# aiola-lab/whisper-medusa

Measured on AMD Instinct MI355X. Metric: decoded_tokens_per_sec, higher is better.
Workload: dtype bf16 + fp16 decoder GEMM operands (one plane; fp32 accumulate)

## Files before the change

whisper-medusa_amd/csrc/wm_decoder.hip:

```cpp
#include "wm_internal.h"
#include <algorithm>
#include <cstdlib>
#include <type_traits>
#include "wm_skinny_gemm.h"
#include "wm_select.h"

__global__ void k_embed(float* __restrict__ h, const bf16_t* __restrict__ tok_emb, const float* __restrict__ pos_emb,
                        const int* __restrict__ base, const int* __restrict__ tok_src, int tok_stride, int use_base_off,
                        int Mper, int d, int V, int Tmax, const int* __restrict__ depth,
                        const int4* __restrict__ rowinfo = nullptr, const int* __restrict__ ids = nullptr, int ids_stride = 0,
                        const float* __restrict__ gnext = nullptr, bf16_t* __restrict__ xo = nullptr, size_t xplane = 0,
                        float2* __restrict__ stats = nullptr, int sld = 0)
{
    const int row = blockIdx.x;
    int s = row / Mper, r = row - s * Mper;
    bool base_row = false;
    int b0;
    if (rowinfo) {
        const int4 ri = rowinfo[row];
        if (ri.w == 0) return;
        s = ri.x; r = ri.y; b0 = ri.z; base_row = ri.w == 1;
    } else {
        b0 = base[s];
    }
// ... 374 lines not shown
    typedef unsigned long long u64;
    float M = -INFINITY, L = 0.f; float4 acc = make_float4(0.f, 0.f, 0.f, 0.f);

    for (int sp = sp0; sp < sp1; ++sp) {
        AttnAcc st;
        st.m_run = -INFINITY; st.l_run = 0.f;
#pragma unroll
        for (int dt = 0; dt < 4; ++dt) st.o[dt] = f32x4_t{0.f, 0.f, 0.f, 0.f};
        if (CROSS) {
            const int nkb = (sp + 1) * 256 + w * 64, nkend = (sp + 1 < sp1) ? min(S, nkb + 64) : 0;
            if (aw && kb < kend) attn_block64(st, kv_widen(c0), kv_widen(c1), qhi, qlo, kb, g, limit, kb + 32 < kend);
            if constexpr (KV8) {
                if (aw && nkb < nkend) kv_load8(c0, kp8, vp8, nkb, c, g, lane);
                if (aw && nkb + 32 < nkend) kv_load8(c1, kp8, vp8, nkb + 32, c, g, lane);
            } else {
                if (aw && nkb < nkend) kv_load<NT>(c0, kp, vp, nkb, c, g, lane);
                if (aw && nkb + 32 < nkend) kv_load<NT>(c1, kp, vp, nkb + 32, c, g, lane);
            }
            kb = nkb; kend = nkend;
        } else {
            for (; kb < kend; kb += 128) {
                const bool second = CROSS ? false : ((kb >> 7) & 1);
                if constexpr (!KV8) {
                    if (kb + 128 < kend) { if (second) kv_load<NT>(c0, kp, vp, kb + 128, c, g, lane); else kv_load<NT>(c1, kp, vp, kb + 128, c, g, lane); }
                    if (second) attn_step(st, c1, qhi, qlo, kb, g, limit, b0, anc); else attn_step(st, c0, qhi, qlo, kb, g, limit, b0, anc);
                }
            }
        }
        const float m_run = st.m_run, l_run = st.l_run;
        const f32x4_t (&o)[4] = st.o;
        if (aw) {
            if (g == 0) { s_m[w][c] = m_run; s_l[w][c] = l_run; }
#pragma unroll
            for (int dt = 0; dt < 4; ++dt)
                *reinterpret_cast<float4*>(&s_o[w][c][dt * 16 + 4 * g]) = make_float4(o[dt][0], o[dt][1], o[dt][2], o[dt][3]);
        }
        __syncthreads();
        M = -INFINITY; L = 0.f; acc = make_float4(0.f, 0.f, 0.f, 0.f);
        if (qr < rows) {
            M = fmaxf(fmaxf(s_m[0][qr], s_m[1][qr]), fmaxf(s_m[2][qr], s_m[3][qr]));
#pragma unroll
            for (int ww = 0; ww < 4; ++ww) {
                const float e = (s_m[ww][qr] == -INFINITY) ? 0.f : __expf(s_m[ww][qr] - M);
                L += s_l[ww][qr] * e;
                const float4 ov = *reinterpret_cast<const float4*>(&s_o[ww][qr][ch]);
                acc.x += ov.x * e; acc.y += ov.y * e; acc.z += ov.z * e; acc.w += ov.w * e;
            }
        }
        if (!CROSS) break;
        if (qr < rows) {
            *reinterpret_cast<float4*>(&s_part[sp - sp0][qr][ch]) = acc;
            if (ch == 0) { s_part[sp - sp0][qr][64] = M; s_part[sp - sp0][qr][65] = L; }
            if (gx > 1) {
                u64* pd = reinterpret_cast<u64*>(po + (((size_t)row * H + hd) * NS + sp) * 64 + ch);
                __hip_atomic_store(pd, ((u64)__float_as_uint(acc.y) << 32) | __float_as_uint(acc.x), __ATOMIC_RELAXED, __HIP_MEMORY_SCOPE_AGENT);
                __hip_atomic_store(pd + 1, ((u64)__float_as_uint(acc.w) << 32) | __float_as_uint(acc.z), __ATOMIC_RELAXED, __HIP_MEMORY_SCOPE_AGENT);
                if (ch == 0)
                    __hip_atomic_store(reinterpret_cast<u64*>(ml + (((size_t)row * H + hd) * NS + sp) * 2),
                                       ((u64)__float_as_uint(L) << 32) | __float_as_uint(M), __ATOMIC_RELAXED, __HIP_MEMORY_SCOPE_AGENT);
            }
        }
        if (sp + 1 < sp1) __syncthreads();
    }
    TL_MID
    if (!CROSS) {
        if (qr < rows) {
            const float inv = 1.0f / L;
            const size_t oi = packed_index(row, hd * 64 + ch, K32);
            act_st4(xout + oi, xout + xplane + oi, make_float4(acc.x * inv, acc.y * inv, acc.z * inv, acc.w * inv));
        }
        TL_END
        return;
    }
    if (gx > 1) {
        asm volatile("s_waitcnt vmcnt(0)" ::: "memory");
        __syncthreads();
        if (threadIdx.x == 0) {
            const int t = __hip_atomic_fetch_add(ticket + blockIdx.z * H + hd, 1, __ATOMIC_RELAXED, __HIP_MEMORY_SCOPE_AGENT);
            const int last = (t == gx - 1);
            if (last) __hip_atomic_store(ticket + blockIdx.z * H + hd, 0, __ATOMIC_RELAXED, __HIP_MEMORY_SCOPE_AGENT);
            s_last = last;
        }
        __syncthreads();
        if (!s_last) { TL_END return; }
    } else __syncthreads();
    if (qr < rows) {
        float ms[WM_XATTN_NS_MAX], ls[WM_XATTN_NS_MAX]; float4 ov[WM_XATTN_NS_MAX];
        if (gx > 1) {
            const u64* mlp = reinterpret_cast<const u64*>(ml + ((size_t)row * H + hd) * NS * 2);
            const u64* op = reinterpret_cast<const u64*>(po + ((size_t)row * H + hd) * NS * 64 + ch);
            u64 rml[WM_XATTN_NS_MAX], ro0[WM_XATTN_NS_MAX], ro1[WM_XATTN_NS_MAX];
#pragma unroll
            for (int sp = 0; sp < WM_XATTN_NS_MAX; ++sp) {
                const int spc = min(sp, NS - 1);
                rml[sp] = __hip_atomic_load(mlp + spc, __ATOMIC_RELAXED, __HIP_MEMORY_SCOPE_AGENT);
                ro0[sp] = __hip_atomic_load(op + (size_t)spc * 32, __ATOMIC_RELAXED, __HIP_MEMORY_SCOPE_AGENT);
                ro1[sp] = __hip_atomic_load(op + (size_t)spc * 32 + 1, __ATOMIC_RELAXED, __HIP_MEMORY_SCOPE_AGENT);
            }
#pragma unroll
            for (int sp = 0; sp < WM_XATTN_NS_MAX; ++sp) {
                ms[sp] = __uint_as_float((unsigned)rml[sp]); ls[sp] = __uint_as_float((unsigned)(rml[sp] >> 32));
                ov[sp] = make_float4(__uint_as_float((unsigned)ro0[sp]), __uint_as_float((unsigned)(ro0[sp] >> 32)),
                                     __uint_as_float((unsigned)ro1[sp]), __uint_as_float((unsigned)(ro1[sp] >> 32)));
            }
        } else {
#pragma unroll
            for (int sp = 0; sp < WM_XATTN_NS_MAX; ++sp) {
                const int spc = min(sp, NS - 1);
                ms[sp] = s_part[spc][qr][64]; ls[sp] = s_part[spc][qr][65];
                ov[sp] = *reinterpret_cast<const float4*>(&s_part[spc][qr][ch]);
            }
        }
        float Mx = -INFINITY;
#pragma unroll
        for (int sp = 0; sp < WM_XATTN_NS_MAX; ++sp) if (sp < NS) Mx = fmaxf(Mx, ms[sp]);
        float Lt = 0.f; float4 o4 = make_float4(0.f, 0.f, 0.f, 0.f);
#pragma unroll
        for (int sp = 0; sp < WM_XATTN_NS_MAX; ++sp) {
            if (sp < NS) {
                const float e = (ms[sp] == -INFINITY) ? 0.f : __expf(ms[sp] - Mx);
                Lt += ls[sp] * e;
                o4.x += ov[sp].x * e; o4.y += ov[sp].y * e; o4.z += ov[sp].z * e; o4.w += ov[sp].w * e;
            }
        }
        const float inv = vsc / Lt;
        const size_t oi = packed_index(row, hd * 64 + ch, K32);
        act_st4(xout + oi, xout + xplane + oi, make_float4(o4.x * inv, o4.y * inv, o4.z * inv, o4.w * inv));
    }
    TL_END
}


__device__ __forceinline__ void sib_block_pop(float (&tv)[6], int (&ti)[6], float* sv, int* si, int tid, float& mx, int& mi)
{
    const int lane = tid & 63, w = tid >> 6;
    mx = tv[0]; mi = ti[0];
#pragma unroll
    for (int o = 32; o > 0; o >>= 1) {
        const float ov = __shfl_xor(mx, o, 64); const int oi = __shfl_xor(mi, o, 64);
        if (ov > mx || (ov == mx && oi < mi)) { mx = ov; mi = oi; }
    }
    __syncthreads();
    if (lane == 0) { sv[w] = mx; si[w] = mi; }
    __syncthreads();
    mx = sv[0]; mi = si[0];
#pragma unroll
    for (int q = 1; q < 4; ++q) if (sv[q] > mx || (sv[q] == mx && si[q] < mi)) { mx = sv[q]; mi = si[q]; }
    if (ti[0] == mi && mi != 0x7fffffff) {
#pragma unroll
        for (int q = 0; q < 5; ++q) { tv[q] = tv[q + 1]; ti[q] = ti[q + 1]; }
        tv[5] = -INFINITY; ti[5] = 0x7fffffff;
    }
}
__device__ __forceinline__ void sib_insert(float (&tv)[6], int (&ti)[6], float v, int vi)
{
    if (v > tv[5] || (v == tv[5] && vi < ti[5])) {
#pragma unroll
        for (int j = 0; j < 6; ++j)
            if (v > tv[j] || (v == tv[j] && vi < ti[j])) { const float fv = tv[j]; const int fi = ti[j]; tv[j] = v; ti[j] = vi; v = fv; vi = fi; }
    }
}

template <bool NEED_Z, bool TS>
__device__ __forceinline__ void
select1_body(const float* __restrict__ logits, const GenDev& gp, const unsigned char* __restrict__ mask, const float* __restrict__ exppen,
             const int* __restrict__ L, int rps, float* __restrict__ part1, const int4* __restrict__ rowinfo, float2* __restrict__ sibpart,
             const TsDev& ts, int ts_verify)
{
    __shared__ float sv[4]; __shared__ int si[4]; __shared__ float sz[4];
    const int row = blockIdx.y, sp = blockIdx.x;
    int s = row / rps, ri_i = row - s * rps;
    const bool sibrow = sibpart != nullptr && row - s * rps == 1;
    if (rowinfo) {
        const int4 ri = rowinfo[row];
        if (ri.w != 2) return;
        s = ri.x; ri_i = ri.y;
    }
    const int tid = threadIdx.x, lane = tid & 63, w = tid >> 6;
    const int cur_len = L[s];
    const float* x = logits + (size_t)row * gp.Vpad;
    const int per = (gp.V + SEL_SP - 1) / SEL_SP, n0 = sp * per, n1 = min(gp.V, n0 + per);
    int4 rec = make_int4(0, 0, 0, 0);
    if (TS) rec = ts_row_record(gp, ts, ts_verify, s, ri_i, cur_len);
    extern __shared__ unsigned rp_sh[];
    const bool rp = TS && ts.rp != 0;
    if (rp) rp_build(ts, rp_row_prefix(ts, ts_verify, s, ri_i, cur_len), n0, n1, -1, gp.V, rp_sh, tid, 256);
    auto pl = [&](int n) {
        float v = x[n];
        if (rp) v = rp_pen(v, n, n0, ts, rp_sh);
        v = proc_logit(v, n, cur_len, gp, mask, exppen);
        if (TS) v = ts_mask(v, n, rec, gp, ts);
        if (rp && rp_banned(n, n0, gp.V, rp_sh)) v = -INFINITY;
        return v;
    };
    float mx = -INFINITY; int mi = 0x7fffffff;
    if (sibrow) {
        float tv[6]; int ti[6];
#pragma unroll
        for (int j = 0; j < 6; ++j) { tv[j] = -INFINITY; ti[j] = 0x7fffffff; }
        for (int n = n0 + tid; n < n1; n += 256) sib_insert(tv, ti, pl(n), n);
        float2* mine = sibpart + ((size_t)s * SEL_SP + sp) * 6;
        float m0 = -INFINITY; int i0 = 0x7fffffff;
        for (int j = 0; j < 6; ++j) {
            float pm; int pi;
            sib_block_pop(tv, ti, sv, si, tid, pm, pi);
            if (j == 0) { m0 = pm; i0 = pi; }
            if (tid == 0) mine[j] = make_float2(pm, __int_as_float(pi));
        }
        __syncthreads();
        mx = m0; mi = i0;
    } else if (!TS) {
        for (int n = n0 + tid; n < n1; n += 256) {
            const float v = proc_logit(x[n], n, cur_len, gp, mask, exppen);
            if (v > mx || (v == mx && n < mi)) { mx = v; mi = n; }
        }
#pragma unroll
        for (int o = 32; o > 0; o >>= 1) {
            const float ov = __shfl_xor(mx, o, 64); const int oi = __shfl_xor(mi, o, 64);
            if (ov > mx || (ov == mx && oi < mi)) { mx = ov; mi = oi; }
        }
        if (lane == 0) { sv[w] = mx; si[w] = mi; }
        __syncthreads();
        mx = sv[0]; mi = si[0];
#pragma unroll
        for (int k = 1; k < 4; ++k) if (sv[k] > mx || (sv[k] == mx && si[k] < mi)) { mx = sv[k]; mi = si[k]; }
    }
    if (TS) {
        float mt = -INFINITY, ms = -INFINITY; int it = 0x7fffffff, is = 0x7fffffff;
        for (int n = n0 + tid; n < n1; n += 256) {
            const float v = pl(n);
            if (n < ts.tb) { if (v > mt || (v == mt && n < it)) { mt = v; it = n; } }
            else if (v > ms || (v == ms && n < is)) { ms = v; is = n; }
        }
        block_argmax(mt, it, sv, si, tid);
        block_argmax(ms, is, sv, si, tid);
        float zt = 0.f, zs = 0.f, zs1 = 0.f;
        for (int n = (NEED_Z ? n0 : max(n0, ts.tb)) + tid; n < n1; n += 256) {
            const float v = pl(n);
            if (v == -INFINITY) continue;
            if (n < ts.tb) zt += expf((v - mt) * gp.inv_temp);
            else { if (NEED_Z) zs += expf((v - ms) * gp.inv_temp); zs1 += expf(v - ms); }
        }
        zt = block_sum(zt, sz, tid); zs = block_sum(zs, sz, tid); zs1 = block_sum(zs1, sz, tid);
        if (tid == 0) {
            float* o = part1 + ((size_t)row * SEL_SP + sp) * 4;
            o[0] = mt; o[1] = __int_as_float(it); o[2] = zt;
            float* q = ts.part1t + ((size_t)row * SEL_SP + sp) * 4;
            q[0] = ms; q[1] = __int_as_float(is); q[2] = zs; q[3] = zs1;
        }
        return;
    }
    float z = 0.f;
    if (NEED_Z && mx != -INFINITY)
        for (int n = n0 + tid; n < n1; n += 256) {
            const float v = proc_logit(x[n], n, cur_len, gp, mask, exppen);
            z += (v == -INFINITY) ? 0.f : expf((v - mx) * gp.inv_temp);
        }
    z = wave_sum(z);
    if (lane == 0) sz[w] = z;
    __syncthreads();
    if (tid == 0) {
        float* o = part1 + ((size_t)row * SEL_SP + sp) * 4;
        o[0] = mx; o[1] = __int_as_float(mi); o[2] = (sz[0] + sz[1]) + (sz[2] + sz[3]);
    }
}

template <bool NEED_Z = true>
__global__ void __launch_bounds__(256)
k_select1(const float* __restrict__ logits, GenDev gp, const unsigned char* __restrict__ mask, const float* __restrict__ exppen,
          const int* __restrict__ L, int rps, float* __restrict__ part1, const int4* __restrict__ rowinfo = nullptr,
          float2* __restrict__ sibpart = nullptr)
{
    select1_body<NEED_Z, false>(logits, gp, mask, exppen, L, rps, part1, rowinfo, sibpart, TsDev{}, 0);
}
template <bool NEED_Z>
__global__ void __launch_bounds__(256)
k_select1_ts(const float* __restrict__ logits, GenDev gp, const unsigned char* __restrict__ mask, const float* __restrict__ exppen,
             const int* __restrict__ L, int rps, float* __restrict__ part1, const int4* __restrict__ rowinfo, float2* __restrict__ sibpart,
             TsDev ts, int ts_verify)
{
    select1_body<NEED_Z, true>(logits, gp, mask, exppen, L, rps, part1, rowinfo, sibpart, ts, ts_verify);
}

template <bool TS>
__device__ __forceinline__ void
select2_body(const float* __restrict__ logits, const GenDev& gp, const unsigned char* __restrict__ mask, const float* __restrict__ exppen,
             const int* __restrict__ L, const int* __restrict__ cand, int rps, int out_row0, const float* __restrict__ part1,
             float* __restrict__ part2, int* __restrict__ amax, float* __restrict__ pc, const TreeDev* __restrict__ tree,
             const int4* __restrict__ rowinfo, const TsDev& ts)
{
    __shared__ float sh[4];
    const int row = blockIdx.y, sp = blockIdx.x;
    int s = row / rps, i = row - s * rps;
    if (rowinfo) {
        const int4 ri = rowinfo[row];
        if (ri.w != 2) return;
        s = ri.x; i = ri.y;
    }
    const int tid = threadIdx.x, lane = tid & 63, w = tid >> 6;
    const int cur_len = L[s];
    const float* x = logits + (size_t)row * gp.Vpad;
    const float* p1 = part1 + (size_t)row * SEL_SP * 4;
    float mx = -INFINITY; int mi = 0x7fffffff;
    float invz;
    int4 rec = make_int4(0, 0, 0, 0); int forced = 0;
    if (TS) {
        const TsSel f = ts_finish(p1, ts.part1t + (size_t)row * SEL_SP * 4, gp.inv_temp);
        mx = f.mx; mi = f.mi; invz = 1.0f / f.z; forced = f.forced;
        rec = ts_row_record(gp, ts, 1, s, i, cur_len);
    } else {
#pragma unroll
        for (int k = 0; k < SEL_SP; ++k) {
            const float v = p1[4 * k]; const int idx = __float_as_int(p1[4 * k + 1]);
            if (v > mx || (v == mx && idx < mi)) { mx = v; mi = idx; }
        }
        float z = 0.f;
#pragma unroll
        for (int k = 0; k < SEL_SP; ++k) {
            const float v = p1[4 * k];
            z += (v == -INFINITY) ? 0.f : p1[4 * k + 2] * expf((v - mx) * gp.inv_temp);
        }
        invz = 1.0f / z;
    }
    const int per = (gp.V + SEL_SP - 1) / SEL_SP, n0 = sp * per, n1 = min(gp.V, n0 + per);
    extern __shared__ unsigned rp_sh[];
    const bool rp = TS && ts.rp != 0;
    const int probe = (TS && i + 1 < rps) ? cand[s * WM_CAND_STRIDE + i + 1] : -1;
    if (rp) rp_build(ts, rp_row_prefix(ts, 1, s, i, cur_len), n0, n1, probe, gp.V, rp_sh, tid, 256);
    auto pl = [&](int n) {
        float v = x[n];
        if (rp) v = rp_pen(v, n, n0, ts, rp_sh);
        v = proc_logit(v, n, cur_len, gp, mask, exppen);
        if (TS) { v = ts_mask(v, n, rec, gp, ts); if (forced && n < ts.tb) v = -INFINITY; }
        if (rp && rp_banned(n, n0, gp.V, rp_sh)) v = -INFINITY;
        return v;
    };
    auto pl_probe = [&](int n) {
        float v = x[n];
        if (rp && (rp_sh[0] & 1u)) v = rp_penalise(v, ts.rp_pen);
        v = proc_logit(v, n, cur_len, gp, mask, exppen);
        if (TS) { v = ts_mask(v, n, rec, gp, ts); if (forced && n < ts.tb) v = -INFINITY; }
        if (rp && (rp_sh[0] & 2u)) v = -INFINITY;
        return v;
    };
    float hs = 0.f;
    for (int n = n0 + tid; n < n1; n += 256) {
        const float v = pl(n);
        const float p = (v == -INFINITY) ? 0.f : expf((v - mx) * gp.inv_temp) * invz;
        hs += p * logf(p + 1e-5f);
    }
    hs = wave_sum(hs);
    if (lane == 0) sh[w] = hs;
    __syncthreads();
    if (tid == 0) {
        const int orow = out_row0 + row;
        part2[(size_t)orow * SEL_SP + sp] = (sh[0] + sh[1]) + (sh[2] + sh[3]);
        if (sp == 0) {
            amax[orow] = mi;
            if (TS) ts.forced[orow] = forced;
            if (tree) {
                if (i == 0) pc[out_row0 + s * rps] = 0.f;
                for (int j = 0; j < 4; ++j) {
                    const int ch = tree->children[i][j];
                    if (ch < 0) break;
                    const int c = cand[s * WM_CAND_STRIDE + ch];
                    const float vc = proc_logit(x[c], c, cur_len, gp, mask, exppen);
                    pc[out_row0 + s * rps + ch] = (vc == -INFINITY) ? 0.f : expf((vc - mx) * gp.inv_temp) * invz;
                }
            } else {
                float pcv = 0.f;
                if (i + 1 < rps) {
                    const int c = cand[s * WM_CAND_STRIDE + i + 1];
                    const float vc = pl_probe(c);
                    pcv = (vc == -INFINITY) ? 0.f : expf((vc - mx) * gp.inv_temp) * invz;
                }
                pc[orow] = pcv;
            }
        }
    }
}

__global__ void __launch_bounds__(256)
k_select2(const float* __restrict__ logits, GenDev gp, const unsigned char* __restrict__ mask, const float* __restrict__ exppen,
          const int* __restrict__ L, const int* __restrict__ cand, int rps, int out_row0, const float* __restrict__ part1,
          float* __restrict__ part2, int* __restrict__ amax, float* __restrict__ pc, const TreeDev* __restrict__ tree,
          const int4* __restrict__ rowinfo = nullptr)
{
    select2_body<false>(logits, gp, mask, exppen, L, cand, rps, out_row0, part1, part2, amax, pc, tree, rowinfo, TsDev{});
}
__global__ void __launch_bounds__(256)
k_select2_ts(const float* __restrict__ logits, GenDev gp, const unsigned char* __restrict__ mask, const float* __restrict__ exppen,
             const int* __restrict__ L, const int* __restrict__ cand, int rps, int out_row0, const float* __restrict__ part1,
             float* __restrict__ part2, int* __restrict__ amax, float* __restrict__ pc, const int4* __restrict__ rowinfo, TsDev ts)
{
    select2_body<true>(logits, gp, mask, exppen, L, cand, rps, out_row0, part1, part2, amax, pc, nullptr, rowinfo, ts);
}

__global__ void k_select_argmax(const float* __restrict__ part1, int nrows, int out_row0, int* __restrict__ amax)
{
    const int row = blockIdx.x * blockDim.x + threadIdx.x;
    if (row >= nrows) return;
    const float* p1 = part1 + (size_t)row * SEL_SP * 4;
    float mx = -INFINITY; int mi = 0x7fffffff;
    for (int k = 0; k < SEL_SP; ++k) {
        const float v = p1[4 * k]; const int idx = __float_as_int(p1[4 * k + 1]);
        if (v > mx || (v == mx && idx < mi)) { mx = v; mi = idx; }
    }
    amax[out_row0 + row] = mi;
}
__global__ void k_select_argmax_ts(const float* __restrict__ part1, int nrows, int out_row0, int* __restrict__ amax, TsDev ts)
{
    const int row = blockIdx.x * blockDim.x + threadIdx.x;
    if (row >= nrows) return;
    const TsSel f = ts_finish(part1 + (size_t)row * SEL_SP * 4, ts.part1t + (size_t)row * SEL_SP * 4, 1.0f);
    amax[out_row0 + row] = f.mi;
    ts.forced[out_row0 + row] = f.forced;
}

__global__ void k_rows_take_carried(float* __restrict__ dst, const float* __restrict__ keep, const int* __restrict__ carry, int d, int M,
                                    const int* __restrict__ done)
{
    if (done && *done) return;
    const int m = blockIdx.x;
    if (m >= M || !carry[m]) return;
    const float4* sp = reinterpret_cast<const float4*>(keep + (size_t)m * d);
    float4* dp = reinterpret_cast<float4*>(dst + (size_t)m * d);
    for (int j = threadIdx.x; j < (d >> 2); j += blockDim.x) dp[j] = sp[j];
}

template <bool TS>
__device__ __forceinline__ void
cand_fin_body(const float* __restrict__ part1, const GenDev& gp, int* __restrict__ amax, int* __restrict__ cand, const float2* __restrict__ sibpart,
              const TsDev& ts)
{
    __shared__ float sv[4]; __shared__ int si[4];
    const int s = blockIdx.x, tid = threadIdx.x, rps = gp.K + 1;
    if (tid < rps) {
        const float* p1 = part1 + (size_t)(s * rps + tid) * SEL_SP * 4;
        float mx = -INFINITY; int mi = 0x7fffffff;
        if (TS) mi = ts_finish(p1, ts.part1t + (size_t)(s * rps + tid) * SEL_SP * 4, 1.0f).mi;
        else
            for (int k = 0; k < SEL_SP; ++k) {
                const float v = p1[4 * k]; const int idx = __float_as_int(p1[4 * k + 1]);
                if (v > mx || (v == mx && idx < mi)) { mx = v; mi = idx; }
            }
        amax[s * rps + tid] = mi;
        cand[s * WM_CAND_STRIDE + tid] = mi;
    }
    if (TS) {
        __syncthreads();
        if (tid == 0 && ts.on) {
            int4 st = ts.st[s];
            const int len = ts.L[s];
            for (int i = 0; i < rps; ++i) {
                st = ts_fold(st, cand[s * WM_CAND_STRIDE + i], ts.tb);
                ts.ver[s * WM_CAND_STRIDE + i] = ts_record(st, len + i + 1, gp.begin, ts.tb, gp.V, ts.mit);
            }
        }
    }
    if (gp.sib <= 0 || sibpart == nullptr) return;
    float tv[6]; int ti[6];
#pragma unroll
    for (int j = 0; j < 6; ++j) { tv[j] = -INFINITY; ti[j] = 0x7fffffff; }
    if (tid < SEL_SP * 6) {
        const float2 p = sibpart[(size_t)s * SEL_SP * 6 + tid];
        tv[0] = p.x; ti[0] = __float_as_int(p.y);
    }
    for (int j = 0; j <= gp.sib; ++j) {
        float mx; int mi;
        sib_block_pop(tv, ti, sv, si, tid, mx, mi);
        if (tid == 0 && j > 0) cand[s * WM_CAND_STRIDE + gp.K + j] = (mi == 0x7fffffff) ? -1 : mi;
    }
}

__global__ void __launch_bounds__(256)
k_cand_fin(const float* __restrict__ part1, GenDev gp, int* __restrict__ amax, int* __restrict__ cand, const float2* __restrict__ sibpart)
{
    cand_fin_body<false>(part1, gp, amax, cand, sibpart, TsDev{});
}
__global__ void __launch_bounds__(256)
k_cand_fin_ts(const float* __restrict__ part1, GenDev gp, int* __restrict__ amax, int* __restrict__ cand, const float2* __restrict__ sibpart,
              TsDev ts)
{
    cand_fin_body<true>(part1, gp, amax, cand, sibpart, ts);
}

__global__ void __launch_bounds__(256)
k_step_begin(const int* __restrict__ carry, const int* __restrict__ L, const int* __restrict__ kvlen, const int* __restrict__ finished,
             int4* __restrict__ rowinfo, int4* __restrict__ sinfo, int* __restrict__ steprows, int rps, int B, int Rmax)
{
    __shared__ int s_start[1025];
    if (threadIdx.x == 0) {
        int acc = 0;
        for (int s = 0; s < B; ++s) { s_start[s] = acc; acc += finished[s] ? 0 : (carry[s] ? rps : 1); }
        s_start[B] = acc;
        steprows[0] = acc; steprows[1] = (acc + 15) >> 4;
        if (acc > 0) steprows[2] += 1;
    }
    __syncthreads();
    const int nrows = s_start[B];
    for (int s = threadIdx.x; s < B; s += blockDim.x) {
        const int m = carry[s] ? 1 : 0, cnt = finished[s] ? 0 : (m ? rps : 1), pb = m ? L[s] : kvlen[s], r0 = s_start[s];
        sinfo[s] = make_int4(r0, cnt, pb, m);
        for (int r = 0; r < cnt; ++r) rowinfo[r0 + r] = make_int4(s, r, pb, m ? 2 : 1);
    }
    for (int row = nrows + threadIdx.x; row < Rmax; row += blockDim.x) rowinfo[row] = make_int4(0, 0, 0, 0);
}

template <bool TS>
__device__ __forceinline__ void
accept_body(const GenDev& gp, const int* __restrict__ cand, const int* __restrict__ amax, const float* __restrict__ pc,
            const float* __restrict__ part2, int* __restrict__ ids, int* __restrict__ L, int* __restrict__ kvlen,
            int* __restrict__ finished, int* __restrict__ niter, long long* __restrict__ hist, int* __restrict__ done, int B,
            int* __restrict__ carry, const float* __restrict__ hf, float* __restrict__ hf_keep, int d,
            int* __restrict__ hostflags, const float* __restrict__ hb, float* __restrict__ hb_keep,
            const int4* __restrict__ sinfo, int* __restrict__ sel_src, int* __restrict__ sel_n, int* __restrict__ sel_base, const TsDev& ts)
{
    const int s = blockIdx.x, lane = threadIdx.x;
    if (finished[s]) { if (sel_n && lane == 0) sel_n[s] = 0; return; }
    const int K = gp.K, rps = K + 1;
    const int row0 = sinfo ? sinfo[s].x : s * rps;
    if (sinfo != nullptr && sinfo[s].w == 0) {
        const float4* srcp = reinterpret_cast<const float4*>(hf + (size_t)row0 * d);
        float4* dstp = reinterpret_cast<float4*>(hf_keep + (size_t)s * d);
        for (int j = lane; j < (d >> 2); j += 64) dstp[j] = srcp[j];
        if (hb) {
            const float4* bs = reinterpret_cast<const float4*>(hb + (size_t)row0 * d);
            float4* bd = reinterpret_cast<float4*>(hb_keep + (size_t)s * d);
            for (int j = lane; j < (d >> 2); j += 64) bd[j] = bs[j];
        }
        if (lane == 0) { kvlen[s] = L[s]; carry[s] = 1; }
        return;
    }
    bool ok = false;
    if (lane < K) {
        if (gp.accept_mode == WM_ACCEPT_GREEDY) ok = (cand[s * WM_CAND_STRIDE + lane + 1] == amax[row0 + lane]);
        else {
            const float* hp = part2 + (size_t)(row0 + lane) * SEL_SP;
            float hsum = 0.f;
#pragma unroll
            for (int k = 0; k < SEL_SP; ++k) hsum += hp[k];
            const float thr = fminf(gp.thr, gp.alpha * expf(hsum));
            ok = pc[row0 + lane] > thr;
        }
    }
    const unsigned long long m = __ballot(ok);
    const unsigned long long inv = ~m;
    int a = (inv == 0ull) ? 64 : (__ffsll((long long)inv) - 1);
    if (a > K) a = K;
    if (gp.force_accept >= 0) a = min(gp.force_accept, K);
    const int Lcur = L[s];
    const int n_emit = (a == 0) ? 2 : a + 1;
    int tok = -1;
    if (lane < n_emit) {
        tok = (a == 0 && lane == 1) ? amax[row0] : cand[s * WM_CAND_STRIDE + lane];
        if (Lcur + lane < gp.Tids) ids[(size_t)s * gp.Tids + Lcur + lane] = tok;
    }
    const bool hit_eos = __ballot(lane < n_emit && tok == gp.eos) != 0ull;
    int sib_row = -1;
    if (gp.sib > 0 && carry != nullptr && a == 0 && sel_n != nullptr && gp.force_accept < 0) {
        const int nxt = amax[row0];
        const unsigned long long hit = __ballot(lane < gp.sib && cand[s * WM_CAND_STRIDE + rps + lane] == nxt);
        if (hit) sib_row = rps + (__ffsll((long long)hit) - 1);
    }
    const bool do_carry = carry != nullptr && (a > 0 || sib_row >= 0);
    const int crow = (a > 0) ? a : sib_row;
    if (do_carry) {
        const float4* srcp = reinterpret_cast<const float4*>(hf + (size_t)(row0 + crow) * d);
        float4* dstp = reinterpret_cast<float4*>(hf_keep + (size_t)s * d);
        for (int j = lane; j < (d >> 2); j += 64) dstp[j] = srcp[j];
        if (hb) {
            const float4* bs = reinterpret_cast<const float4*>(hb + (size_t)(row0 + crow) * d);
            float4* bd = reinterpret_cast<float4*>(hb_keep + (size_t)s * d);
            for (int j = lane; j < (d >> 2); j += 64) bd[j] = bs[j];
        }
    }
    if (sel_n != nullptr && lane < 16) sel_src[s * 16 + lane] = (lane == 1 && sib_row >= 0) ? sib_row : lane;
    if (lane == 0) {
        const int Ln = Lcur + n_emit;
        if (TS && ts.on) {
            int4 st = ts.st[s];
            for (int j = 0; j < n_emit; ++j) st = ts_fold(st, (a == 0 && j == 1) ? amax[row0] : cand[s * WM_CAND_STRIDE + j], ts.tb);
            ts.st[s] = st;
        }
        L[s] = Ln;
        kvlen[s] = (a == 0 && sib_row < 0) ? Lcur + 1 : (do_carry ? Ln : Lcur + a);
        if (carry) carry[s] = do_carry ? 1 : 0;
        if (sel_n != nullptr) { sel_n[s] = sib_row >= 0 ? 2 : 0; sel_base[s] = Lcur; }
        if (sib_row >= 0) atomicAdd(reinterpret_cast<unsigned long long*>(hist + 17), 1ull);
// ... 935 lines not shown
```

whisper-medusa_amd/csrc/wm_select.h:

```cpp
#pragma once
#include "wm_internal.h"

#define SEL_SP 16

__device__ __forceinline__ float proc_logit(float x, int n, int cur_len, const GenDev& gp, const unsigned char* mask,
                                            const float* exppen)
{
    if (n == gp.eos && gp.exp_start >= 0 && cur_len > gp.exp_start) x += fabsf(x) * exppen[cur_len];
    const unsigned char mk = mask[n];
    if ((mk & 1) || ((mk & 2) && cur_len == gp.begin)) x = -INFINITY;
    return x;
}

__device__ __forceinline__ float ts_mask(float v, int n, int4 rec, const GenDev& gp, const TsDev& ts)
{
    if (n == ts.nots) return -INFINITY;
    if (n >= ts.tb) return (n < rec.x || n > rec.y) ? -INFINITY : v;
    return ((rec.z & 2) || ((rec.z & 1) && n < gp.eos)) ? -INFINITY : v;
}
__device__ __forceinline__ int4 ts_row_record(const GenDev& gp, const TsDev& ts, int ts_verify, int s, int i, int cur_len)
{
    if (!ts.on) return make_int4(0, 0, 0, 0);
    return ts_verify ? ts.ver[s * WM_CAND_STRIDE + i] : ts_record(ts.st[s], cur_len, gp.begin, ts.tb, gp.V, ts.mit);
}

struct RpPre { const int* pre; int len; const int* ext; int next; };
__host__ __device__ __forceinline__ int rp_words(int V) { return V / (32 * SEL_SP) + 3; }
static inline size_t rp_lds_bytes(const TsDev& ts, int V) { return ts.rp ? (size_t)(4 + 2 * rp_words(V)) * sizeof(unsigned) : 0; }
__device__ __forceinline__ int rp_tok(const RpPre& p, int j) { return j < p.len ? p.pre[j] : p.ext[j - p.len]; }
__device__ __forceinline__ void rp_build(const TsDev& ts, const RpPre& p, int n0, int n1, int probe, int V, unsigned* sh, int tid, int nthr)
{
    const int W = rp_words(V);
    for (int k = tid; k < 4 + 2 * W; k += nthr) sh[k] = 0u;
    __syncthreads();
    const int T = p.len + p.next, g = ts.rp_g;
    for (int j = tid; j < T; j += nthr) {
        const int tok = rp_tok(p, j);
        const bool in = tok >= n0 && tok < n1;
        unsigned fl = 0u;
        if (ts.rp & 1) {
            fl |= 1u;
            if (in) atomicOr(&sh[4 + ((tok - n0) >> 5)], 1u << ((tok - n0) & 31));
        }
        if ((ts.rp & 2) && T >= g && j >= g - 1) {
            bool same = true;
            for (int k = 1; k < g && same; ++k) same = rp_tok(p, j - k) == rp_tok(p, T - k);
            if (same) {
                fl |= 2u;
                if (in) atomicOr(&sh[4 + W + ((tok - n0) >> 5)], 1u << ((tok - n0) & 31));
            }
        }
        if (tok == probe && fl) atomicOr(&sh[0], fl);
    }
    __syncthreads();
}
__device__ __forceinline__ float rp_penalise(float x, float p) { return x < 0.f ? x * p : __fdiv_rn(x, p); }
__device__ __forceinline__ float rp_pen(float x, int n, int n0, const TsDev& ts, const unsigned* sh)
{
    return ((sh[4 + ((n - n0) >> 5)] >> ((n - n0) & 31)) & 1u) ? rp_penalise(x, ts.rp_pen) : x;
}
__device__ __forceinline__ bool rp_banned(int n, int n0, int V, const unsigned* sh)
{
    return (sh[4 + rp_words(V) + ((n - n0) >> 5)] >> ((n - n0) & 31)) & 1u;
}
__device__ __forceinline__ RpPre rp_row_prefix(const TsDev& ts, int verify, int s, int i, int cur_len)
{
    if (ts.rp_len) return RpPre{ts.rp_ids + (size_t)i * ts.rp_stride, ts.rp_len[i], ts.rp_ids, 0};
    return RpPre{ts.rp_ids + (size_t)s * ts.rp_stride, min(cur_len, ts.rp_stride), ts.rp_cand + s * WM_CAND_STRIDE, verify ? i + 1 : 0};
}
struct TsSel { float mx; int mi; float z; int forced; };
__device__ __forceinline__ TsSel ts_finish(const float* p1, const float* p1t, float inv_temp)
{
    float mt = -INFINITY, ms = -INFINITY; int it = 0x7fffffff, is = 0x7fffffff;
    for (int k = 0; k < SEL_SP; ++k) {
        const float v = p1[4 * k]; const int idx = __float_as_int(p1[4 * k + 1]);
        if (v > mt || (v == mt && idx < it)) { mt = v; it = idx; }
        const float u = p1t[4 * k]; const int iu = __float_as_int(p1t[4 * k + 1]);
        if (u > ms || (u == ms && iu < is)) { ms = u; is = iu; }
    }
    float zt = 0.f, zs = 0.f, zs1 = 0.f;
    for (int k = 0; k < SEL_SP; ++k) {
        const float v = p1[4 * k], u = p1t[4 * k];
        if (v != -INFINITY) zt += p1[4 * k + 2] * expf((v - mt) * inv_temp);
        if (u != -INFINITY) { zs += p1t[4 * k + 2] * expf((u - ms) * inv_temp); zs1 += p1t[4 * k + 3] * expf(u - ms); }
    }
    TsSel r;
    r.forced = (ms != -INFINITY && ms + logf(zs1) > mt) ? 1 : 0;
    if (r.forced) { r.mx = ms; r.mi = is; r.z = zs; }
    else if (ms > mt) { r.mx = ms; r.mi = is; r.z = zs + (mt == -INFINITY ? 0.f : zt * expf((mt - ms) * inv_temp)); }
    else { r.mx = mt; r.mi = it; r.z = zt + (ms == -INFINITY ? 0.f : zs * expf((ms - mt) * inv_temp)); }
    return r;
}
__device__ __forceinline__ void block_argmax(float& mx, int& mi, float* sv, int* si, int tid)
{
    const int lane = tid & 63, w = tid >> 6;
#pragma unroll
    for (int o = 32; o > 0; o >>= 1) {
        const float ov = __shfl_xor(mx, o, 64); const int oi = __shfl_xor(mi, o, 64);
        if (ov > mx || (ov == mx && oi < mi)) { mx = ov; mi = oi; }
    }
    __syncthreads();
    if (lane == 0) { sv[w] = mx; si[w] = mi; }
    __syncthreads();
    mx = sv[0]; mi = si[0];
#pragma unroll
    for (int k = 1; k < 4; ++k) if (sv[k] > mx || (sv[k] == mx && si[k] < mi)) { mx = sv[k]; mi = si[k]; }
}
__device__ __forceinline__ float block_sum(float z, float* sz, int tid)
{
    z = wave_sum(z);
    __syncthreads();
    if ((tid & 63) == 0) sz[tid >> 6] = z;
    __syncthreads();
    return (sz[0] + sz[1]) + (sz[2] + sz[3]);
}
```

Baseline: 1564.

## Add batched register-resident select paths with DPP/permlane argmax reductions

Adds fast paths for the non-TS select1, select2 and candidate-finish kernels. Each thread loads up to 16 logits and mask bytes into registers up front, then runs the per-row processing, argmax, softmax-normaliser and entropy work on those registers. Wave argmax now uses permlane swaps and DPP instead of shuffles, and block reductions use double-buffered shared slots, which cuts __syncthreads per round. This is meant to reduce memory latency and barrier overhead in the small-batch sampling kernels, at the cost of higher register pressure and a second code path that must match the original tie-breaking semantics.

```diff
diff --git a/whisper-medusa_amd/csrc/wm_decoder.hip b/whisper-medusa_amd/csrc/wm_decoder.hip
--- a/whisper-medusa_amd/csrc/wm_decoder.hip
+++ b/whisper-medusa_amd/csrc/wm_decoder.hip
@@ -550,6 +550,16 @@
         tv[5] = -INFINITY; ti[5] = 0x7fffffff;
     }
 }
+__device__ __forceinline__ void sib_block_pop_v(float (&tv)[6], int (&ti)[6], float (*sv)[4], int (*si)[4], int round, int tid, float& mx, int& mi)
+{
+    mx = tv[0]; mi = ti[0];
+    sel_block_argmax(mx, mi, sv, si, round, tid);
+    if (ti[0] == mi && mi != 0x7fffffff) {
+#pragma unroll
+        for (int q = 0; q < 5; ++q) { tv[q] = tv[q + 1]; ti[q] = ti[q + 1]; }
+        tv[5] = -INFINITY; ti[5] = 0x7fffffff;
+    }
+}
 __device__ __forceinline__ void sib_insert(float (&tv)[6], int (&ti)[6], float v, int vi)
 {
     if (v > tv[5] || (v == tv[5] && vi < ti[5])) {
@@ -557,6 +567,62 @@
         for (int j = 0; j < 6; ++j)
             if (v > tv[j] || (v == tv[j] && vi < ti[j])) { const float fv = tv[j]; const int fi = ti[j]; tv[j] = v; ti[j] = vi; v = fv; vi = fi; }
     }
+}
+
+template <bool NEED_Z>
+__device__ __forceinline__ void
+select1_batched(const float* __restrict__ x, const GenDev& gp, const unsigned char* __restrict__ mask, const float* __restrict__ exppen,
+                const int* __restrict__ Ls, float* __restrict__ o, float2* __restrict__ mine, int n0, int n1, float* sz)
+{
+    __shared__ float sv[2][4]; __shared__ int si[2][4];
+    const int tid = threadIdx.x, lane = tid & 63, w = tid >> 6;
+    float v[SEL_EPT]; unsigned mk[SEL_EPT];
+    sel_batch_issue(v, mk, x, mask, n0, gp.V, tid);
+    const int cur_len = *Ls;
+    const float pen = sel_eos_pen(gp, cur_len, exppen);
+#pragma unroll
+    for (int k = 0; k < SEL_EPT; ++k) {
+        const int n = n0 + tid + 256 * k;
+        v[k] = proc_logit_v(v[k], n, mk[k], cur_len, gp, pen);
+    }
+    float mx = -INFINITY; int mi = 0x7fffffff;
+    if (mine) {
+        float tv[6]; int ti[6];
+#pragma unroll
+        for (int j = 0; j < 6; ++j) { tv[j] = -INFINITY; ti[j] = 0x7fffffff; }
+#pragma unroll
+        for (int k = 0; k < SEL_EPT; ++k) {
+            const int n = n0 + tid + 256 * k;
+            if (n < n1) sib_insert(tv, ti, v[k], n);
+        }
+        float m0 = -INFINITY; int i0 = 0x7fffffff;
+        for (int j = 0; j < 6; ++j) {
+            float pm; int pi;
+            sib_block_pop_v(tv, ti, sv, si, j, tid, pm, pi);
+            if (j == 0) { m0 = pm; i0 = pi; }
+            if (tid == 0) mine[j] = make_float2(pm, __int_as_float(pi));
+        }
+        mx = m0; mi = i0;
+    } else {
+#pragma unroll
+        for (int k = 0; k < SEL_EPT; ++k) {
+            const int n = n0 + tid + 256 * k;
+            if (n < n1 && (v[k] > mx || (v[k] == mx && n < mi))) { mx = v[k]; mi = n; }
+        }
+        sel_block_argmax(mx, mi, sv, si, 0, tid);
+    }
+    float z = 0.f;
+    if (NEED_Z && mx != -INFINITY) {
+#pragma unroll
+        for (int k = 0; k < SEL_EPT; ++k) {
+            const int n = n0 + tid + 256 * k;
+            if (n < n1) z += (v[k] == -INFINITY) ? 0.f : expf((v[k] - mx) * gp.inv_temp);
+        }
+    }
+    z = wave_sum(z);
+    if (lane == 0) sz[w] = z;
+    __syncthreads();
+    if (tid == 0) { o[0] = mx; o[1] = __int_as_float(mi); o[2] = (sz[0] + sz[1]) + (sz[2] + sz[3]); }
 }
 
 template <bool NEED_Z, bool TS>
@@ -575,9 +641,16 @@
         s = ri.x; ri_i = ri.y;
     }
     const int tid = threadIdx.x, lane = tid & 63, w = tid >> 6;
-    const int cur_len = L[s];
     const float* x = logits + (size_t)row * gp.Vpad;
     const int per = (gp.V + SEL_SP - 1) / SEL_SP, n0 = sp * per, n1 = min(gp.V, n0 + per);
+    if constexpr (!TS) {
+        if (sel_batched(per)) {
+            select1_batched<NEED_Z>(x, gp, mask, exppen, L + s, part1 + ((size_t)row * SEL_SP + sp) * 4,
+                                    sibrow ? sibpart + ((size_t)s * SEL_SP + sp) * 6 : nullptr, n0, n1, sz);
+            return;
+        }
+    }
+    const int cur_len = L[s];
     int4 rec = make_int4(0, 0, 0, 0);
     if (TS) rec = ts_row_record(gp, ts, ts_verify, s, ri_i, cur_len);
     extern __shared__ unsigned rp_sh[];
@@ -680,6 +753,70 @@
     select1_body<NEED_Z, true>(logits, gp, mask, exppen, L, rps, part1, rowinfo, sibpart, ts, ts_verify);
 }
 
+__device__ __forceinline__ void
+select2_batched(const float* __restrict__ x, const GenDev& gp, const unsigned char* __restrict__ mask, const float* __restrict__ exppen,
+                const int* __restrict__ Ls, const int* __restrict__ cand_s, int rps, int i, int orow, int srow0, const float* __restrict__ p1,
+                float* __restrict__ part2, int* __restrict__ amax, float* __restrict__ pc, const TreeDev* __restrict__ tree, int sp, int n0, int n1,
+                float* sh)
+{
+    const int tid = threadIdx.x, lane = tid & 63, w = tid >> 6;
+    const int ci = cand_s[min(i + 1, rps - 1)];
+    float v[SEL_EPT]; unsigned mk[SEL_EPT];
+    sel_batch_issue(v, mk, x, mask, n0, gp.V, tid);
+    const int cur_len = *Ls;
+    const float4 pq = sel_partials_issue(p1, lane);
+    const int cc = min(max(ci, 0), gp.V - 1);
+    const float xc = x[cc]; const unsigned mc = mask[cc];
+    const float pen = sel_eos_pen(gp, cur_len, exppen);
+    float mx = -INFINITY; int mi = 0x7fffffff;
+#pragma unroll
+    for (int k = 0; k < SEL_SP; ++k) {
+        const float u = sel_lane_f(pq.x, k); const int idx = __float_as_int(sel_lane_f(pq.y, k));
+        if (u > mx || (u == mx && idx < mi)) { mx = u; mi = idx; }
+    }
+    const float zk = (pq.x == -INFINITY) ? 0.f : pq.z * expf((pq.x - mx) * gp.inv_temp);
+    float z = 0.f;
+#pragma unroll
+    for (int k = 0; k < SEL_SP; ++k) z += sel_lane_f(zk, k);
+    const float invz = 1.0f / z;
+    float hs = 0.f;
+#pragma unroll
+    for (int k = 0; k < SEL_EPT; ++k) {
+        const int n = n0 + tid + 256 * k;
+        if (n < n1) {
+            const float u = proc_logit_v(v[k], n, mk[k], cur_len, gp, pen);
+            const float p = (u == -INFINITY) ? 0.f : expf((u - mx) * gp.inv_temp) * invz;
+            hs += p * logf(p + 1e-5f);
+        }
+    }
+    hs = wave_sum(hs);
+    if (lane == 0) sh[w] = hs;
+    __syncthreads();
+    if (tid == 0) {
+        part2[(size_t)orow * SEL_SP + sp] = (sh[0] + sh[1]) + (sh[2] + sh[3]);
+        if (sp == 0) {
+            amax[orow] = mi;
+            if (tree) {
+                if (i == 0) pc[srow0] = 0.f;
+                for (int j = 0; j < 4; ++j) {
+                    const int ch = tree->children[i][j];
+                    if (ch < 0) break;
+                    const int c = cand_s[ch];
+                    const float vc = proc_logit(x[c], c, cur_len, gp, mask, exppen);
+                    pc[srow0 + ch] = (vc == -INFINITY) ? 0.f : expf((vc - mx) * gp.inv_temp) * invz;
+                }
+            } else {
+                float pcv = 0.f;
+                if (i + 1 < rps) {
+                    const float vc = proc_logit_v(xc, ci, mc, cur_len, gp, pen);
+                    pcv = (vc == -INFINITY) ? 0.f : expf((vc - mx) * gp.inv_temp) * invz;
+                }
+                pc[orow] = pcv;
+            }
+        }
+    }
+}
+
 template <bool TS>
 __device__ __forceinline__ void
 select2_body(const float* __restrict__ logits, const GenDev& gp, const unsigned char* __restrict__ mask, const float* __restrict__ exppen,
@@ -696,9 +833,17 @@
         s = ri.x; i = ri.y;
     }
     const int tid = threadIdx.x, lane = tid & 63, w = tid >> 6;
-    const int cur_len = L[s];
     const float* x = logits + (size_t)row * gp.Vpad;
     const float* p1 = part1 + (size_t)row * SEL_SP * 4;
+    if constexpr (!TS) {
+        const int per = (gp.V + SEL_SP - 1) / SEL_SP;
+        if (sel_batched(per)) {
+            select2_batched(x, gp, mask, exppen, L + s, cand + s * WM_CAND_STRIDE, rps, i, out_row0 + row, out_row0 + s * rps, p1, part2, amax, pc, tree,
+                            sp, sp * per, min(gp.V, sp * per + per), sh);
+            return;
+        }
+    }
+    const int cur_len = L[s];
     float mx = -INFINITY; int mi = 0x7fffffff;
     float invz;
     int4 rec = make_int4(0, 0, 0, 0); int forced = 0;
@@ -833,6 +978,37 @@
 {
     __shared__ float sv[4]; __shared__ int si[4];
     const int s = blockIdx.x, tid = threadIdx.x, rps = gp.K + 1;
+    if constexpr (!TS) {
+        const bool sib = gp.sib > 0 && sibpart != nullptr;
+        const float4* p4 = reinterpret_cast<const float4*>(part1 + (size_t)(s * rps + min(tid, rps - 1)) * SEL_SP * 4);
+        float4 pp[SEL_SP];
+#pragma unroll
+        for (int k = 0; k < SEL_SP; ++k) pp[k] = p4[k];
+        float2 sp6 = make_float2(-INFINITY, __int_as_float(0x7fffffff));
+        if (sib) sp6 = sibpart[(size_t)s * SEL_SP * 6 + min(tid, SEL_SP * 6 - 1)];
+        if (tid < rps) {
+            float mx = -INFINITY; int mi = 0x7fffffff;
+#pragma unroll
+            for (int k = 0; k < SEL_SP; ++k) {
+                const float v = pp[k].x; const int idx = __float_as_int(pp[k].y);
+                if (v > mx || (v == mx && idx < mi)) { mx = v; mi = idx; }
+            }
+            amax[s * rps + tid] = mi;
+            cand[s * WM_CAND_STRIDE + tid] = mi;
+        }
+        if (!sib) return;
+        float tv[6]; int ti[6];
+#pragma unroll
+        for (int j = 0; j < 6; ++j) { tv[j] = -INFINITY; ti[j] = 0x7fffffff; }
+        if (tid < SEL_SP * 6) { tv[0] = sp6.x; ti[0] = __float_as_int(sp6.y); }
+        __shared__ float sv2[2][4]; __shared__ int si2[2][4];
+        for (int j = 0; j <= gp.sib; ++j) {
+            float mx; int mi;
+            sib_block_pop_v(tv, ti, sv2, si2, j, tid, mx, mi);
+            if (tid == 0 && j > 0) cand[s * WM_CAND_STRIDE + gp.K + j] = (mi == 0x7fffffff) ? -1 : mi;
+        }
+        return;
+    }
     if (tid < rps) {
         const float* p1 = part1 + (size_t)(s * rps + tid) * SEL_SP * 4;
         float mx = -INFINITY; int mi = 0x7fffffff;
diff --git a/whisper-medusa_amd/csrc/wm_select.h b/whisper-medusa_amd/csrc/wm_select.h
--- a/whisper-medusa_amd/csrc/wm_select.h
+++ b/whisper-medusa_amd/csrc/wm_select.h
@@ -10,6 +10,75 @@
     const unsigned char mk = mask[n];
     if ((mk & 1) || ((mk & 2) && cur_len == gp.begin)) x = -INFINITY;
     return x;
+}
+__device__ __forceinline__ bool sel_eos_pen_on(const GenDev& gp, int cur_len) { return gp.exp_start >= 0 && cur_len > gp.exp_start; }
+__device__ __forceinline__ float sel_eos_pen(const GenDev& gp, int cur_len, const float* exppen)
+{
+    return sel_eos_pen_on(gp, cur_len) ? exppen[cur_len] : 0.f;
+}
+__device__ __forceinline__ float proc_logit_v(float x, int n, unsigned mk, int cur_len, const GenDev& gp, float pen)
+{
+    if (n == gp.eos && sel_eos_pen_on(gp, cur_len)) x += fabsf(x) * pen;
+    if ((mk & 1) || ((mk & 2) && cur_len == gp.begin)) x = -INFINITY;
+    return x;
+}
+
+#define SEL_EPT 16
+__device__ __forceinline__ bool sel_batched(int per) { return per <= 256 * SEL_EPT; }
+__device__ __forceinline__ void sel_batch_issue(float (&xv)[SEL_EPT], unsigned (&mk)[SEL_EPT], const float* __restrict__ x,
+                                                const unsigned char* __restrict__ mask, int n0, int V, int tid)
+{
+#pragma unroll
+    for (int k = 0; k < SEL_EPT; ++k) {
+        const int n = min(n0 + tid + 256 * k, V - 1);
+        xv[k] = x[n]; mk[k] = mask[n];
+    }
+}
+__device__ __forceinline__ float4 sel_partials_issue(const float* __restrict__ p1, int lane)
+{
+    return reinterpret_cast<const float4*>(p1)[lane & (SEL_SP - 1)];
+}
+__device__ __forceinline__ float sel_lane_f(float v, int k) { return __int_as_float(__builtin_amdgcn_readlane(__float_as_int(v), k)); }
+
+__device__ __forceinline__ void sel_better(float& mx, int& mi, float ov, int oi)
+{
+    if (ov > mx || (ov == mx && oi < mi)) { mx = ov; mi = oi; }
+}
+template <int CTRL>
+__device__ __forceinline__ void sel_dpp_step(float& mx, int& mi)
+{
+    const float ov = __int_as_float(__builtin_amdgcn_update_dpp(0, __float_as_int(mx), CTRL, 0xf, 0xf, false));
+    const int oi = __builtin_amdgcn_update_dpp(0, mi, CTRL, 0xf, 0xf, false);
+    sel_better(mx, mi, ov, oi);
+}
+__device__ __forceinline__ void sel_wave_argmax(float& mx, int& mi)
+{
+    {
+        const auto a = __builtin_amdgcn_permlane32_swap(__float_as_uint(mx), __float_as_uint(mx), false, false);
+        const auto b = __builtin_amdgcn_permlane32_swap((unsigned)mi, (unsigned)mi, false, false);
+        mx = __uint_as_float(a[0]); mi = (int)b[0];
+        sel_better(mx, mi, __uint_as_float(a[1]), (int)b[1]);
+    }
+    {
+        const auto a = __builtin_amdgcn_permlane16_swap(__float_as_uint(mx), __float_as_uint(mx), false, false);
+        const auto b = __builtin_amdgcn_permlane16_swap((unsigned)mi, (unsigned)mi, false, false);
+        mx = __uint_as_float(a[0]); mi = (int)b[0];
+        sel_better(mx, mi, __uint_as_float(a[1]), (int)b[1]);
+    }
+    sel_dpp_step<0x140>(mx, mi);
+    sel_dpp_step<0x141>(mx, mi);
+    sel_dpp_step<0x4e>(mx, mi);
+    sel_dpp_step<0xb1>(mx, mi);
+}
+__device__ __forceinline__ void sel_block_argmax(float& mx, int& mi, float (*sv)[4], int (*si)[4], int round, int tid)
+{
+    sel_wave_argmax(mx, mi);
+    float* v = sv[round & 1]; int* ix = si[round & 1];
+    if ((tid & 63) == 0) { v[tid >> 6] = mx; ix[tid >> 6] = mi; }
+    __syncthreads();
+    mx = v[0]; mi = ix[0];
+#pragma unroll
+    for (int q = 1; q < 4; ++q) sel_better(mx, mi, v[q], ix[q]);
 }
 
 __device__ __forceinline__ float ts_mask(float v, int n, int4 rec, const GenDev& gp, const TsDev& ts)
```

Measured after the change: 1563. No clear change (-0.1%).
